# cloneofsimo/paint-with-words-sd

Measured on AMD Instinct MI355X. Metric: 512x512 images/sec (30 steps, CFG) SD1.5+PwW, higher is better.
Workload: dtype bf16

## Files before the change

__graft_entry__.py:

```python
import os
import sys

REPO = os.path.dirname(os.path.abspath(__file__))
PKG = os.path.join(REPO, "paint-with-words-sd_amd")
for p in (PKG, REPO, os.path.join(REPO, "tests")):
    if p not in sys.path:
        sys.path.insert(0, p)


def build():
    import build as pww_build
    lib = pww_build.build_lib(verbose=False)
    exe = pww_build.build_native_check()
    import pww_hip
    import paint_with_words
    handle = pww_hip.load_library()
    missing = [n for n in pww_hip.EXPORTS if not hasattr(handle, n)]
    assert not missing, "libpww_hip.so lacks %s" % missing
    from pww_hip import _lib
    built = [(lib, handle.pww_version())]
    for name in pww_build.SIDE_LIBS:
        path = pww_build.build_side(name)
        side = _lib.load_side(name)
        assert side is not None, "%s was not built" % path
        missing = [n for n in _lib.side_spec(name)["exports"] if not hasattr(side, n)]
        assert not missing, "%s lacks %s" % (os.path.basename(path), missing)
        built.append((path, getattr(side, "pww_%s_version" % name)()))
    print("built %s and %s" % (", ".join("%s (ABI %d)" % b for b in built), exe))


def smoke():
    import math
    import numpy as np
    import torch
    import pww_hip
    from oracle import pww_oracle as O
    import pww_cases as cases

    assert torch.cuda.is_available(), "smoke() needs a HIP device"
    dev = torch.device("cuda:0")
    print("device arch:", pww_hip.device_arch())

    case = cases.make_attention_case("sd15_n1024")
    dtype = torch.float16
    mod = case["attn_cross"].to(dev, dtype)
    hidden = case["hidden"].to(dev, dtype)
    wf = lambda w, sigma, qk: 0.4 * w * math.log(1 + sigma) * qk.max()
    ctx = {"CONTEXT_TENSOR": case["ctx"].to(dev, dtype), "CROSS_ATTENTION_WEIGHT_1024": case["w"].to(dev),
           "SIGMA": torch.tensor(7.84), "WEIGHT_FUNCTION": wf}
    y = pww_hip.inj_forward(mod, hidden, ctx).float().cpu()
# ... 35 lines not shown
```

paint-with-words-sd_amd/build.py:

```python
import os
import subprocess
import sys

HERE = os.path.dirname(os.path.abspath(__file__))
REPO = os.path.dirname(HERE)
CSRC = os.path.join(HERE, "csrc")
LIB = os.path.join(HERE, "pww_hip", "libpww_hip.so")
LIB_EXPERIMENTS = os.path.join(HERE, "pww_hip", "libpww_hip_experiments.so")
UNITS = [("pww_api.hip", [], ""), ("pww_attn.hip", [], ""), ("pww_cross.hip", [], ""), ("pww_cross_lean.hip", [], ""), ("pww_reduce.hip", [], ""),
         ("pww_mask.hip", [], ""), ("pww_qproj.hip", [], ""), ("pww_norm.hip", [], ""), ("pww_blocks.hip", [], ""), ("pww_conv.hip", [], ""), ("pww_probs.hip", [], ""),
         ("pww_attn_inst.hip", ["-DPWW_INST_F16"], ".f16"), ("pww_attn_inst.hip", ["-DPWW_INST_BF16"], ".bf16"),
         ("pww_cross_inst.hip", ["-DPWW_INST_F16", "-DPWW_INST_NW=2"], ".f16.nw2"), ("pww_cross_inst.hip", ["-DPWW_INST_F16", "-DPWW_INST_NW=4"], ".f16.nw4"),
         ("pww_cross_inst.hip", ["-DPWW_INST_BF16", "-DPWW_INST_NW=2"], ".bf16.nw2"), ("pww_cross_inst.hip", ["-DPWW_INST_BF16", "-DPWW_INST_NW=4"], ".bf16.nw4")]
EXPERIMENT_UNITS = [("pww_cross_out.hip", [], "")]
_ATTN_HEADERS = ["pww_tile.h", "pww_attn_core.h", "pww_cross_tile.h"]
SIDE_FLAGS = ["-fvisibility=hidden"]
SIDE_LIBS = {
    "long": ("pww_long.hip", _ATTN_HEADERS, "the long-prompt launches"),
    "scope": ("pww_scope.hip", _ATTN_HEADERS, "cross-attention with per-head / per-row score statistics"),
    "linear": ("pww_linear.hip", [], "linear layers with a bias / residual / GEGLU epilogue"),
    "regions": ("pww_regions.hip", [], "region masks and the per-pixel blend of the noise predictions"),
    "lora": ("pww_lora.hip", [], "the per-row low-rank update of unmerged LoRA adapters"),
}
SOURCES = sorted({u[0] for u in UNITS + EXPERIMENT_UNITS})
HEADERS = ["pww_common.h", "pww_tile.h", "pww_attn_core.h", "pww_attn_kernel.h", "pww_cross_tile.h", "pww_cross_kernel.h", os.path.join(REPO, "include", "pww_hip.h")]
SIDE_PATHS = {n: os.path.join(HERE, "pww_hip", "libpww_hip_%s.so" % n) for n in SIDE_LIBS}
SIDE_UNITS = {n: [(v[0], SIDE_FLAGS, "")] for n, v in SIDE_LIBS.items()}
LIB_LONG, LIB_SCOPE, LIB_LINEAR, LIB_REGIONS, LIB_LORA = (SIDE_PATHS[n] for n in ("long", "scope", "linear", "regions", "lora"))
LONG_UNITS, SCOPE_UNITS, LINEAR_UNITS, REGIONS_UNITS, LORA_UNITS = (SIDE_UNITS[n] for n in ("long", "scope", "linear", "regions", "lora"))
HIPCC = os.environ.get("HIPCC", "/opt/rocm/bin/hipcc")
FLAGS = ["--offload-arch=gfx950", "-O3", "-std=c++17", "-fPIC", "-Wall",
         "-Wno-unused-function", "-mllvm", "-amdgpu-kernarg-preload-count=16"]


PER_FILE_FLAGS = {"pww_mask.hip": ["-ffp-contract=off"], "pww_regions.hip": ["-ffp-contract=off"]}


def _newer(target, deps):
    if not os.path.exists(target):
        return True
    t = os.path.getmtime(target)
    return any(os.path.getmtime(d) > t for d in deps)


def _deps():
    return ([os.path.join(CSRC, s) for s in SOURCES] + [h if os.path.isabs(h) else os.path.join(CSRC, h) for h in HEADERS] + [__file__])


def _build(lib, units, defines, objdir, verbose, jobs=None):
    os.makedirs(objdir, exist_ok=True)
    order = sorted(units, key=lambda u: {"pww_cross_inst.hip": 0, "pww_attn_inst.hip": 1, "pww_cross_lean.hip": 2}.get(u[0], 3))
    jobs = jobs or max(2, min(len(order), os.cpu_count() or 4, int(os.environ.get("MAX_JOBS", 16))))
# ... 12 lines not shown
        if p.returncode != 0:
            for _, q in running:
                q.kill()
            raise RuntimeError("hipcc failed: %s\n%s" % (" ".join(cmd), out))
        if verbose and out.strip():
            print(out)
    subprocess.run([HIPCC, "--offload-arch=gfx950", "-shared", "-fPIC", "-s"] + sorted(objs) + ["-o", lib], check=True)
    return lib


def build_lib(force=False, verbose=False):
    if not force and not _newer(LIB, _deps()):
        return LIB
    return _build(LIB, UNITS, [], os.path.join(HERE, "build"), verbose)


def build_experiments(force=False, verbose=False):
    if not force and not _newer(LIB_EXPERIMENTS, _deps()):
        return LIB_EXPERIMENTS
    return _build(LIB_EXPERIMENTS, UNITS + EXPERIMENT_UNITS, ["-DPWW_EXPERIMENTS=1"], os.path.join(HERE, "build", "experiments"), verbose)


def build_side(name, force=False, verbose=False):
    unit, headers, _ = SIDE_LIBS[name]
    lib = SIDE_PATHS[name]
    deps = [os.path.join(CSRC, f) for f in [unit, "pww_common.h", "pww_side_host.h"] + headers] + [os.path.join(REPO, "include", h) for h in ("pww_hip.h", "pww_hip_%s.h" % name)] + [__file__]
    if not force and not _newer(lib, deps):
        return lib
    return _build(lib, SIDE_UNITS[name], [], os.path.join(HERE, "build", name), verbose)


def build_long(force=False, verbose=False): return build_side("long", force, verbose)
def build_scope(force=False, verbose=False): return build_side("scope", force, verbose)
def build_linear(force=False, verbose=False): return build_side("linear", force, verbose)
def build_regions(force=False, verbose=False): return build_side("regions", force, verbose)
def build_lora(force=False, verbose=False): return build_side("lora", force, verbose)


def _build_check(exe, lib, libname, defines, force):
    src = os.path.join(REPO, "tests", "native", "attn_check.cpp")
    if not force and not _newer(exe, [src, lib, os.path.join(REPO, "include", "pww_hip.h")]):
        return exe
    cmd = [HIPCC, "--offload-arch=gfx950", "-O2", "-std=c++17"] + defines + [src, "-o", exe, "-L" + os.path.dirname(lib), "-l" + libname,
                                                                              "-Wl,-rpath,$ORIGIN/../../paint-with-words-sd_amd/pww_hip"]
    subprocess.run(cmd, check=True)
    return exe


def build_native_check(force=False):
    return _build_check(os.path.join(REPO, "tests", "native", "attn_check"), build_lib(), "pww_hip", [], force)


def build_native_check_experiments(force=False):
    return _build_check(os.path.join(REPO, "tests", "native", "attn_check_experiments"), build_experiments(), "pww_hip_experiments", ["-DPWW_EXPERIMENTS=1"], force)


if __name__ == "__main__":
    force = "--force" in sys.argv
    print(build_lib(force=force, verbose=True))
    print(build_native_check(force=force))
    for name in SIDE_LIBS:
        print(build_side(name, force=force, verbose=True))
    if "--experiments" in sys.argv:
        print(build_experiments(force=force, verbose=True))
        print(build_native_check_experiments(force=force))
```

paint-with-words-sd_amd/pww_hip/_lib.py:

```python
import ctypes
import os

_HERE = os.path.dirname(os.path.abspath(__file__))
LIB_PATH = os.environ.get("PWW_HIP_LIB", os.path.join(_HERE, "libpww_hip.so"))
EXPERIMENTS_LIB_PATH = os.environ.get("PWW_HIP_EXPERIMENTS_LIB", os.path.join(_HERE, "libpww_hip_experiments.so"))

LONG_LIB_PATH = os.environ.get("PWW_HIP_LONG_LIB", os.path.join(_HERE, "libpww_hip_long.so"))
SCOPE_LIB_PATH = os.environ.get("PWW_HIP_SCOPE_LIB", os.path.join(_HERE, "libpww_hip_scope.so"))
LINEAR_LIB_PATH = os.environ.get("PWW_HIP_LINEAR_LIB", os.path.join(_HERE, "libpww_hip_linear.so"))
REGIONS_LIB_PATH = os.environ.get("PWW_HIP_REGIONS_LIB", os.path.join(_HERE, "libpww_hip_regions.so"))
LORA_LIB_PATH = os.environ.get("PWW_HIP_LORA_LIB", os.path.join(_HERE, "libpww_hip_lora.so"))

PWW_OK, PWW_EINVAL, PWW_ENOTSUP, PWW_EHIP = 0, -22, -95, -5
MIN_VERSION = 127
DTYPE_F16, DTYPE_BF16 = 0, 1
LAYOUT_NCHW, LAYOUT_NHWC = 0, 1
ACT_NONE, ACT_SILU = 0, 1
LINEAR_NONE, LINEAR_BIAS, LINEAR_BIAS_RESIDUAL, LINEAR_BIAS_GEGLU = 0, 1, 2, 3
MAX_HEAD_DIM = 160

EXPORTS = ("pww_version", "pww_has_experiments", "pww_last_error", "pww_device_arch", "pww_self_attn_fwd", "pww_cross_attn_fwd",
           "pww_cross_attn_fwd_stat", "pww_cross_attn_fwd_stat_ex",
           "pww_qk_reduce", "pww_mask_build", "pww_mask_build_rgb", "pww_mask_build_f32", "pww_resize_tokens", "pww_gauss_blur", "pww_inpaint_prep", "pww_cfg_combine", "pww_store_f32",
           "pww_workspace_bytes", "pww_profile_arm", "pww_profile_elapsed_us", "pww_profile_reset", "pww_debug_timeline", "pww_debug_path_counts",
           "pww_debug_last_attn_route",
           "pww_qproj_stat", "pww_qproj_parts", "pww_cross_attn_fwd_parts", "pww_mask_build_f32_levels", "pww_qk_parts", "pww_qk_parts_count",
           "pww_group_norm_fwd", "pww_group_norm_workspace_bytes", "pww_add_layer_norm", "pww_add_layer_norm_bias", "pww_geglu", "pww_bias_residual",
           "pww_conv3x3_workspace_bytes", "pww_conv3x3_fwd", "pww_cross_attn_probs")
EXPERIMENT_EXPORTS = ("pww_cross_attn_fwd_fused", "pww_cross_attn_fwd_fused_ex", "pww_cross_fused_workspace_bytes", "pww_cross_fused_state_bytes",
                      "pww_cross_attn_fwd_parts_out", "pww_cross_attn_out_supported")


LONG_EXPORTS = ("pww_long_version", "pww_long_last_error", "pww_long_qk_parts", "pww_long_qk_parts_count", "pww_long_cross_attn_fwd_parts",
                "pww_long_cross_attn_probs", "pww_long_profile_arm", "pww_long_profile_elapsed_us")
LONG_MIN_VERSION = 100
LONG_MIN_KEYS, LONG_MAX_KEYS = 129, 256


SCOPE_EXPORTS = ("pww_scope_version", "pww_scope_last_error", "pww_scope_head_parts_count", "pww_scope_head_parts", "pww_scope_cross_attn_fwd")
SCOPE_MIN_VERSION = 100
SCOPE_HEAD, SCOPE_ROW = 1, 2


LINEAR_EXPORTS = ("pww_linear_version", "pww_linear_last_error", "pww_linear_workspace_bytes", "pww_linear_fwd")
LINEAR_MIN_VERSION = 100


REGIONS_EXPORTS = ("pww_regions_version", "pww_regions_last_error", "pww_regions_masks", "pww_regions_combine")
REGIONS_MIN_VERSION = 100
REGIONS_MAX, REGIONS_MAX_PLANE, REGIONS_MAX_FEATHER = 8, 9216, 8.0


LORA_EXPORTS = ("pww_lora_version", "pww_lora_last_error", "pww_lora_fwd")
LORA_MIN_VERSION = 100
LORA_MAX_ADAPTERS, LORA_MAX_RANK, LORA_MAX_SEGMENTS = 8, 128, 3


class AttnDesc(ctypes.Structure):
    _fields_ = [("dtype", ctypes.c_int32), ("B", ctypes.c_int32), ("H", ctypes.c_int32), ("N", ctypes.c_int32),
                ("M", ctypes.c_int32), ("D", ctypes.c_int32),
                ("q_stride", ctypes.c_int64 * 3), ("k_stride", ctypes.c_int64 * 3),
                ("v_stride", ctypes.c_int64 * 3), ("o_stride", ctypes.c_int64 * 3),
                ("scale", ctypes.c_float), ("bias_stride", ctypes.c_int64 * 4)]


class CrossOpts(ctypes.Structure):
    _fields_ = [("size", ctypes.c_uint32), ("bias_cols", ctypes.c_int32), ("coeff_scalar_dev", ctypes.c_void_p),
                ("bias_compact", ctypes.c_void_p), ("col_idx", ctypes.c_void_p), ("R", ctypes.c_int32), ("gated_images", ctypes.c_int32),
                ("compact_stride", ctypes.c_int64 * 2), ("col_idx_stride", ctypes.c_int64)]


class QprojDesc(ctypes.Structure):
    _fields_ = [("dtype", ctypes.c_int32), ("B", ctypes.c_int32), ("N", ctypes.c_int32), ("Cin", ctypes.c_int32), ("H", ctypes.c_int32),
                ("D", ctypes.c_int32), ("M", ctypes.c_int32), ("x_stride", ctypes.c_int64 * 2), ("q_stride", ctypes.c_int64 * 2),
                ("k_stride", ctypes.c_int64 * 2)]


class GnDesc(ctypes.Structure):
    _fields_ = [("dtype", ctypes.c_int32), ("layout", ctypes.c_int32), ("B", ctypes.c_int32), ("C", ctypes.c_int32), ("HW", ctypes.c_int32),
                ("G", ctypes.c_int32), ("eps", ctypes.c_float), ("act", ctypes.c_int32), ("add_stride", ctypes.c_int32), ("_pad", ctypes.c_int32)]
# ... 5 lines not shown


class ConvDesc(ctypes.Structure):
    _fields_ = [("size", ctypes.c_uint32), ("dtype", ctypes.c_int32), ("B", ctypes.c_int32), ("Hin", ctypes.c_int32), ("Win", ctypes.c_int32),
                ("Cin", ctypes.c_int32), ("Cout", ctypes.c_int32), ("stride", ctypes.c_int32), ("upsample", ctypes.c_int32), ("tile_n", ctypes.c_int32),
                ("splitk", ctypes.c_int32), ("_pad", ctypes.c_int32)]


class LinearDesc(ctypes.Structure):
    _fields_ = [("size", ctypes.c_uint32), ("dtype", ctypes.c_int32), ("M", ctypes.c_int32), ("N", ctypes.c_int32), ("K", ctypes.c_int32),
                ("epilogue", ctypes.c_int32), ("x_stride", ctypes.c_int64), ("y_stride", ctypes.c_int64), ("r_stride", ctypes.c_int64),
                ("tile_n", ctypes.c_int32), ("splitk", ctypes.c_int32)]


class ProbsDesc(ctypes.Structure):
    _fields_ = [("size", ctypes.c_uint32), ("images", ctypes.c_int32), ("accumulate", ctypes.c_int32), ("weight", ctypes.c_float),
                ("out_stride", ctypes.c_int64 * 2)]


class LoraDesc(ctypes.Structure):
    _fields_ = [("size", ctypes.c_uint32), ("dtype", ctypes.c_int32), ("R", ctypes.c_int32), ("T", ctypes.c_int32), ("K", ctypes.c_int32),
                ("N", ctypes.c_int32), ("n_seg", ctypes.c_int32), ("rank", ctypes.c_int32), ("n_adapters", ctypes.c_int32), ("_pad", ctypes.c_int32),
                ("x_row_stride", ctypes.c_int64), ("x_tok_stride", ctypes.c_int64), ("y_row_stride", ctypes.c_int64), ("y_tok_stride", ctypes.c_int64)]


class Region(ctypes.Structure):
    _fields_ = [("r", ctypes.c_uint8), ("g", ctypes.c_uint8), ("b", ctypes.c_uint8), ("_pad", ctypes.c_uint8),
                ("strength", ctypes.c_float)]


class PwwHipError(RuntimeError):
    pass


_lib = None
_exp = None


def _bind(lib, experiments):
    vp, i32, i64, f32 = ctypes.c_void_p, ctypes.c_int32, ctypes.c_int64, ctypes.c_float
    lib.pww_version.restype = ctypes.c_int
    if lib.pww_version() // 100 != 1 or lib.pww_version() < MIN_VERSION:
        raise PwwHipError("libpww_hip ABI version %d.%02d is not 1.x >= 1.%02d (rebuild: python paint-with-words-sd_amd/build.py)"
                          % (lib.pww_version() // 100, lib.pww_version() % 100, MIN_VERSION % 100))
    lib.pww_last_error.restype = ctypes.c_char_p
    lib.pww_device_arch.argtypes = [ctypes.c_char_p, ctypes.c_size_t]
# ... 119 lines not shown
SIDE = {
    "long": dict(path="LONG_LIB_PATH", exports=LONG_EXPORTS, min_version=LONG_MIN_VERSION, missing_ok=False, needs="prompts longer than 77 tokens need it", sigs={
        "pww_long_qk_parts": ([_vp, _vp, _vp, _P(AttnDesc), _i32, _i32, _vp, _sz, _vp], _int),
        "pww_long_qk_parts_count": ([_P(AttnDesc)], _i32),
        "pww_long_cross_attn_fwd_parts": ([_vp, _vp, _vp, _vp, _vp, _i32, _f32, _vp, _P(AttnDesc), _vp, _i32, _vp, _P(CrossOpts), _vp], _int),
        "pww_long_cross_attn_probs": ([_vp, _vp, _vp, _vp, _i32, _f64, _f32, _vp, _P(AttnDesc), _P(CrossOpts), _vp, _P(ProbsDesc), _vp], _int),
        "pww_long_profile_arm": ([], _int),
        "pww_long_profile_elapsed_us": ([_P(_f32)], _int)}),
    "scope": dict(path="SCOPE_LIB_PATH", exports=SCOPE_EXPORTS, min_version=SCOPE_MIN_VERSION, missing_ok=True, needs="per-head / per-row score statistics need it", sigs={
        "pww_scope_head_parts_count": ([_P(AttnDesc)], _i32),
        "pww_scope_head_parts": ([_vp, _vp, _vp, _P(AttnDesc), _i32, _vp, _sz, _vp], _int),
        "pww_scope_cross_attn_fwd": ([_vp, _vp, _vp, _vp, _vp, _i32, _i32, _f32, _vp, _P(AttnDesc), _vp, _i32, _vp, _P(CrossOpts), _vp], _int)}),
    "linear": dict(path="LINEAR_LIB_PATH", exports=LINEAR_EXPORTS, min_version=LINEAR_MIN_VERSION, missing_ok=False, needs="linear layers on the native kernel need it", sigs={
        "pww_linear_workspace_bytes": ([_P(LinearDesc)], _sz),
        "pww_linear_fwd": ([_vp, _vp, _vp, _vp, _vp, _P(LinearDesc), _vp, _sz, _vp], _int)}),
    "regions": dict(path="REGIONS_LIB_PATH", exports=REGIONS_EXPORTS, min_version=REGIONS_MIN_VERSION, missing_ok=False, needs="region prompts need it", sigs={
        "pww_regions_masks": ([_vp, _i32, _i32, _vp, _i32, _f32, _vp, _vp], _int),
        "pww_regions_combine": ([_vp, _vp, _vp, _vp, _f32, _vp, _i32, _i32, _i32, _i64, _i32, _vp], _int)}),
}
SIDE_MORE = {
    "lora": dict(path="LORA_LIB_PATH", exports=LORA_EXPORTS, min_version=LORA_MIN_VERSION, missing_ok=False, needs="LoRA adapters on the native kernel need it", sigs={
        "pww_lora_fwd": ([_vp, _vp, _vp, _vp, _vp, _vp, _P(LoraDesc), _vp], _int)}),
}
_side = {}


def side_spec(name):
    return SIDE[name] if name in SIDE else SIDE_MORE[name]


def load_side(name):
    lib = _side.get(name)
    if lib is not None:
        return lib
    spec = side_spec(name)
    path, so, pre = globals()[spec["path"]], "libpww_hip_%s.so" % name, "pww_%s_" % name
    if not os.path.isfile(path):
        if spec["missing_ok"]:
            return None
        raise PwwHipError("%s not found at %s: %s %s" % (so, path, spec["needs"], _HINT))
    try:
        lib = ctypes.CDLL(path)
        getattr(lib, pre + "version").restype = _int
        version = getattr(lib, pre + "version")()
    except (OSError, AttributeError) as e:
        raise PwwHipError("%s at %s cannot be loaded: %s %s" % (so, path, e, _HINT))
    if version // 100 != 1 or version < spec["min_version"]:
        raise PwwHipError("%s ABI version %d is not 1.x >= %d %s" % (so[:-3], version, spec["min_version"], _HINT))
    missing = [n for n in spec["exports"] if not hasattr(lib, n)]
    if missing:
        raise PwwHipError("%s at %s lacks %s %s" % (so, path, missing, _HINT))
# ... 10 lines not shown
    return lib if lib is not None else load_side("long")


def load_scope():
    lib = _side.get("scope")
    return lib if lib is not None else load_side("scope")


def load_linear():
    lib = _side.get("linear")
    return lib if lib is not None else load_side("linear")


def load_regions():
    lib = _side.get("regions")
    return lib if lib is not None else load_side("regions")


def load_lora():
    lib = _side.get("lora")
    return lib if lib is not None else load_side("lora")


class experiments:

    def __enter__(self):
        global _lib
        load()
        self._prev = _lib
        _lib = load_experiments()
        return _lib

    def __exit__(self, *exc):
        global _lib
        _lib = self._prev
        return False


def check(rc, what, lib=None):
    if rc != PWW_OK:
        msg = (lib or load()).pww_last_error().decode("utf-8", "replace")
        raise PwwHipError("%s failed (rc=%d): %s" % (what, rc, msg))


def device_arch():
    buf = ctypes.create_string_buffer(64)
# ... 3 lines not shown
```

paint-with-words-sd_amd/pww_hip/blocks.py:

```python
import os
import types
import warnings

import torch
import torch.nn as nn
import torch.nn.functional as F

from . import ops

FUSED_NORM = os.environ.get("PWW_FUSED_NORM", "1") != "0"
BATCHED_TEMB = os.environ.get("PWW_BATCHED_TEMB", "1") != "0"
FOLD_CONV_BIAS = os.environ.get("PWW_FOLD_CONV_BIAS", "1") != "0"
CONV1X1_AS_LINEAR = os.environ.get("PWW_CONV1X1_AS_LINEAR", "1") != "0"
LINEAR = os.environ.get("PWW_LINEAR", "1")
CONV3X3 = os.environ.get("PWW_CONV3X3", "1") != "0"


_STATS = {k: [0, 0] for k in ("group_norm", "resnet_block", "transformer_block", "geglu", "conv1x1", "conv3x3", "linear")}
_UNRATED = ("conv1x1", "conv3x3", "linear")
_warned = set()


def stats():
    out = {k: {"fused": v[0], "declined": v[1]} for k, v in _STATS.items()}
    rated = [v for k, v in _STATS.items() if k not in _UNRATED]
    tot = sum(v[0] + v[1] for v in rated)
    out["hit_rate"] = (sum(v[0] for v in rated) / tot) if tot else None
    return out


def reset_stats():
    for v in _STATS.values():
        v[0] = v[1] = 0


def _count(op, fused, x=None, reason=None):
    _STATS[op][0 if fused else 1] += 1
    if not fused and FUSED_NORM and torch.is_tensor(x) and x.is_cuda and x.dtype in (torch.float16, torch.bfloat16):
        key = (op, reason)
        if key not in _warned:
            _warned.add(key)
            warnings.warn("pww_hip.blocks: %s call on a HIP %s tensor handed to the stock op (%s); pww_hip.blocks.stats() counts them"
# ... 106 lines not shown
    h = fused_group_norm(self.norm1, input_tensor, act="silu")
    if fold and _conv3x3_route(self.conv1, h):
        h = ops.conv3x3(h, self.conv1.weight)
    else:
        h = _conv_no_bias(self.conv1, h) if fold else self.conv1(h)
    add = None
    if temb is not None and getattr(self, "time_emb_proj", None) is not None:
        slot = self.__dict__.get("_pww_temb_slot")
        if slot is not None and temb.dtype == h.dtype and temb.dim() == 2 and not torch.is_grad_enabled():
            add = slot[0].project(temb)[:, slot[1]:slot[1] + slot[2]]
        else:
            add = self.time_emb_proj(F.silu(temb))
        if add.dtype != h.dtype:
            add = add.to(h.dtype)
    if fold and _takes(h, self.norm2):
        h = ops.group_norm(h, self.norm2.num_groups, self.norm2.weight, self.norm2.bias, self.norm2.eps, add=add, act="silu", pre_bias=self.conv1.bias)
    else:
        if fold:
            h = h + self.conv1.bias[None, :, None, None]
        h = fused_group_norm(self.norm2, h, add=add, act="silu")
    dropout = getattr(self, "dropout", None)
    if dropout is not None:
        h = dropout(h)
    if getattr(self, "conv_shortcut", None) is not None:
        input_tensor = self.conv_shortcut(input_tensor)
    scale = getattr(self, "output_scale_factor", 1.0)
    if fold and input_tensor.dtype == h.dtype and input_tensor.shape == (h.shape[0], self.conv2.out_channels) + h.shape[2:] and _conv3x3_route(self.conv2, h):
        out = ops.conv3x3(h, self.conv2.weight, self.conv2.bias, residual=input_tensor)
    elif fold and input_tensor.dtype == h.dtype and input_tensor.shape[1] % 8 == 0:
        out = ops.bias_residual(input_tensor, _conv_no_bias(self.conv2, h), self.conv2.bias)
    else:
        out = input_tensor + self.conv2(h)
    return out if scale == 1.0 else out / scale


def _is_conv3x3(m):
    return (isinstance(m, nn.Conv2d) and type(m).forward is nn.Conv2d.forward and m.kernel_size == (3, 3) and m.stride in ((1, 1), (2, 2))
            and m.padding == (1, 1) and m.dilation == (1, 1) and m.groups == 1 and m.padding_mode == "zeros")


STOCK_FROM_ROWS = 16384


def _conv3x3_route(conv, x, upsample=False):
    ok = (CONV3X3 and FUSED_NORM and torch.is_tensor(x) and x.dim() == 4 and _is_conv3x3(conv) and not torch.is_autocast_enabled() and not (torch.is_grad_enabled() and (x.requires_grad or conv.weight.requires_grad))
          and (conv.bias is None or conv.bias.dtype == x.dtype) and ops.conv3x3_takes(x, conv.weight, conv.stride[0], upsample)
          and (upsample or x.shape[0] * ((x.shape[2] - 1) // conv.stride[0] + 1) * ((x.shape[3] - 1) // conv.stride[0] + 1) < STOCK_FROM_ROWS))
    _STATS["conv3x3"][0 if ok else 1] += 1
    return ok


def _conv3x3_forward(self, x, *args, **kwargs):
    if not args and not kwargs and _conv3x3_route(self, x):
        return ops.conv3x3(x, self.weight, self.bias, stride=self.stride[0])
    return self._pww_orig_forward(x, *args, **kwargs)


def _upsample_conv(m):
    if getattr(m, "use_conv_transpose", False) or not getattr(m, "use_conv", True):
        return None
    conv = getattr(m, "Conv2d_0", None) if getattr(m, "name", "conv") != "conv" else getattr(m, "conv", None)
    return conv if _is_conv3x3(conv) and conv.stride == (1, 1) and "forward" not in conv.__dict__ and not conv._forward_hooks and not conv._forward_pre_hooks else None


def _upsample_forward(self, *args, **kwargs):
    plain = 1 <= len(args) <= 2 and set(kwargs) <= {"output_size"} and all(a is None for a in list(args[1:]) + list(kwargs.values()))
    x = args[0] if plain and not (len(args) == 2 and kwargs) else None
    conv = _upsample_conv(self)
    if x is not None and conv is not None and x.dim() == 4 and (getattr(self, "channels", None) in (None, x.shape[1])) and _conv3x3_route(conv, x, upsample=True):
        return ops.conv3x3(x, conv.weight, conv.bias, upsample=True)
    return self._pww_orig_forward(*args, **kwargs)
# ... 148 lines not shown
```

paint-with-words-sd_amd/pww_hip/ops.py:

```python
import ctypes

import torch

from . import _lib
from ._lib import AttnDesc, CrossOpts, ProbsDesc, QprojDesc, Region, PwwHipError

_DT = {torch.float16: _lib.DTYPE_F16, torch.bfloat16: _lib.DTYPE_BF16}


def _stream():
    return ctypes.c_void_p(torch.cuda.current_stream().cuda_stream)


def _ptr(t):
    return ctypes.c_void_p(t.data_ptr()) if t is not None else ctypes.c_void_p(0)


def _require_gpu(*tensors):
    for t in tensors:
        if t is not None and not t.is_cuda:
            raise PwwHipError("pww_hip ops need tensors on a HIP device (got %s); there is no CPU path" % t.device)


def _rows_ok(t):
# ... 919 lines not shown
    B, C, H, W = x.shape
    Cout = weight.shape[0]
    Hv, Wv = H << int(bool(upsample)), W << int(bool(upsample))
    Ho, Wo = (Hv - 1) // stride + 1, (Wv - 1) // stride + 1
    w = _khwc_weight(weight)
    if bias is not None and (bias.dtype != x.dtype or tuple(bias.shape) != (Cout,)):
        raise PwwHipError("conv3x3: bias must be a %s [%d]" % (x.dtype, Cout))
    if bias is not None:
        bias = bias.contiguous()
    if residual is not None:
        if tuple(residual.shape) != (B, Cout, Ho, Wo) or residual.dtype != x.dtype:
            raise PwwHipError("conv3x3: residual must be a %s %s" % (x.dtype, (B, Cout, Ho, Wo)))
        residual = residual.contiguous(memory_format=torch.channels_last)
    d = _lib.ConvDesc(ctypes.sizeof(_lib.ConvDesc), _DT[x.dtype], B, H, W, C, Cout, int(stride), int(bool(upsample)), int(tile_n), int(splitk), 0)
    lib = _lib.load()
    y = torch.empty((B, Cout, Ho, Wo), dtype=x.dtype, device=x.device, memory_format=torch.channels_last)
    nbytes = int(lib.pww_conv3x3_workspace_bytes(ctypes.byref(d)))
    ws = torch.empty(nbytes // 4, dtype=torch.float32, device=x.device) if nbytes else None
    with torch.cuda.device(x.device):
        _lib.check(lib.pww_conv3x3_fwd(_ptr(x), _ptr(w), _ptr(bias), _ptr(residual), _ptr(y), ctypes.byref(d), _ptr(ws), nbytes, _stream()), "pww_conv3x3_fwd")
    return y


def _linear_weight(weight):
    if not torch.is_tensor(weight) or weight.dim() not in (2, 4) or (weight.dim() == 4 and tuple(weight.shape[2:]) != (1, 1)):
        return None
    w = weight.detach().reshape(weight.shape[0], weight.shape[1]) if weight.dim() == 4 else weight.detach()
    return w if w.is_contiguous() and w.data_ptr() == weight.data_ptr() and w.data_ptr() % 16 == 0 else None


def linear_takes(x, weight, geglu=False, bias=None, residual=None, out=None):
    if not (torch.is_tensor(x) and x.is_cuda and x.dtype in _DT and x.dim() >= 2 and torch.is_tensor(weight) and weight.dtype == x.dtype):
        return False
    w = _linear_weight(weight)
    if w is None or x.shape[-1] != w.shape[1] or x.numel() == 0 or _rows(x, "linear") is None:
        return False
    N, K = w.shape
    rows, _, xs = _rows(x, "linear")
    if not (K % 64 == 0 and N % (128 if geglu else 64) == 0 and rows * xs < 2 ** 31 and rows * N < 2 ** 31 and N * K < 2 ** 31):
        return False
    if bias is not None and not (torch.is_tensor(bias) and bias.is_cuda and bias.dtype == x.dtype and tuple(bias.shape) == (N,) and bias.is_contiguous()
                                 and bias.data_ptr() % 8 == 0):
        return False
    shape = tuple(x.shape[:-1]) + (N // 2 if geglu else N,)
    for t in (residual, out):
        if t is not None and not (torch.is_tensor(t) and t.is_cuda and t.dtype == x.dtype and tuple(t.shape) == shape and _rows(t, "linear") is not None):
# ... 100 lines not shown
```

Before: 5.104.

## Fuse ResnetBlock 1x1 conv shortcut into conv2 as extra K-slabs

Adds a new side library with an implicit-GEMM 3x3 conv kernel that treats the 1x1 conv shortcut as additional K-slabs, so conv2 and the shortcut projection are computed in one accumulation with both biases added in the epilogue. This removes the separate shortcut GEMM launch and the write and reread of its output as a residual. It adds split-K with an fp32 workspace and a fold kernel, per-shape tuned tile and split tables, and a routing check in the ResnetBlock forward that falls back to the old path when conditions are not met.

```diff
diff --git a/__graft_entry__.py b/__graft_entry__.py
--- a/__graft_entry__.py
+++ b/__graft_entry__.py
@@ -19,13 +19,18 @@
     assert not missing, "libpww_hip.so lacks %s" % missing
     from pww_hip import _lib
     built = [(lib, handle.pww_version())]
-    for name in pww_build.SIDE_LIBS:
+    def build_side(name):
         path = pww_build.build_side(name)
         side = _lib.load_side(name)
         assert side is not None, "%s was not built" % path
         missing = [n for n in _lib.side_spec(name)["exports"] if not hasattr(side, n)]
         assert not missing, "%s lacks %s" % (os.path.basename(path), missing)
         built.append((path, getattr(side, "pww_%s_version" % name)()))
+
+    for name in pww_build.SIDE_LIBS:
+        build_side(name)
+    for name in pww_build.SIDE_LIBS_CONV:
+        build_side(name)
     print("built %s and %s" % (", ".join("%s (ABI %d)" % b for b in built), exe))
 
 
diff --git a/include/pww_hip_convtail.h b/include/pww_hip_convtail.h
--- /dev/null
+++ b/include/pww_hip_convtail.h
@@ -0,0 +1,30 @@
+#ifndef PWW_HIP_CONVTAIL_H
+#define PWW_HIP_CONVTAIL_H
+
+#include "pww_hip.h"
+
+#ifdef __cplusplus
+extern "C" {
+#endif
+
+#define PWW_CONVTAIL_VERSION 100
+
+int pww_convtail_version(void);
+const char *pww_convtail_last_error(void);
+
+typedef struct pww_convtail_desc {
+    uint32_t size;
+    int32_t dtype;
+    int32_t B, H, W;
+    int32_t Cin, C2, Cout;
+    int32_t tile_n, splitk;
+} pww_convtail_desc_t;
+size_t pww_convtail_workspace_bytes(const pww_convtail_desc_t *desc);
+int pww_convtail_fwd(const void *x, const void *w, const void *x2, const void *w2, const void *bias, const void *bias2, void *y,
+                     const pww_convtail_desc_t *desc, void *workspace, size_t workspace_bytes, void *stream);
+
+#ifdef __cplusplus
+}
+#endif
+
+#endif
diff --git a/paint-with-words-sd_amd/build.py b/paint-with-words-sd_amd/build.py
--- a/paint-with-words-sd_amd/build.py
+++ b/paint-with-words-sd_amd/build.py
@@ -22,12 +22,17 @@
     "regions": ("pww_regions.hip", [], "region masks and the per-pixel blend of the noise predictions"),
     "lora": ("pww_lora.hip", [], "the per-row low-rank update of unmerged LoRA adapters"),
 }
+SIDE_LIBS_CONV = {
+    "convtail": ("pww_conv_tail.hip", [], "conv2 of a ResnetBlock2D with the 1 x 1 shortcut as further K-slabs"),
+}
+ALL_SIDE_LIBS = {**SIDE_LIBS, **SIDE_LIBS_CONV}
 SOURCES = sorted({u[0] for u in UNITS + EXPERIMENT_UNITS})
 HEADERS = ["pww_common.h", "pww_tile.h", "pww_attn_core.h", "pww_attn_kernel.h", "pww_cross_tile.h", "pww_cross_kernel.h", os.path.join(REPO, "include", "pww_hip.h")]
-SIDE_PATHS = {n: os.path.join(HERE, "pww_hip", "libpww_hip_%s.so" % n) for n in SIDE_LIBS}
-SIDE_UNITS = {n: [(v[0], SIDE_FLAGS, "")] for n, v in SIDE_LIBS.items()}
+SIDE_PATHS = {n: os.path.join(HERE, "pww_hip", "libpww_hip_%s.so" % n) for n in ALL_SIDE_LIBS}
+SIDE_UNITS = {n: [(v[0], SIDE_FLAGS, "")] for n, v in ALL_SIDE_LIBS.items()}
 LIB_LONG, LIB_SCOPE, LIB_LINEAR, LIB_REGIONS, LIB_LORA = (SIDE_PATHS[n] for n in ("long", "scope", "linear", "regions", "lora"))
 LONG_UNITS, SCOPE_UNITS, LINEAR_UNITS, REGIONS_UNITS, LORA_UNITS = (SIDE_UNITS[n] for n in ("long", "scope", "linear", "regions", "lora"))
+LIB_CONVTAIL, CONVTAIL_UNITS = SIDE_PATHS["convtail"], SIDE_UNITS["convtail"]
 HIPCC = os.environ.get("HIPCC", "/opt/rocm/bin/hipcc")
 FLAGS = ["--offload-arch=gfx950", "-O3", "-std=c++17", "-fPIC", "-Wall",
          "-Wno-unused-function", "-mllvm", "-amdgpu-kernarg-preload-count=16"]
@@ -86,7 +91,7 @@
 
 
 def build_side(name, force=False, verbose=False):
-    unit, headers, _ = SIDE_LIBS[name]
+    unit, headers, _ = ALL_SIDE_LIBS[name]
     lib = SIDE_PATHS[name]
     deps = [os.path.join(CSRC, f) for f in [unit, "pww_common.h", "pww_side_host.h"] + headers] + [os.path.join(REPO, "include", h) for h in ("pww_hip.h", "pww_hip_%s.h" % name)] + [__file__]
     if not force and not _newer(lib, deps):
@@ -99,6 +104,7 @@
 def build_linear(force=False, verbose=False): return build_side("linear", force, verbose)
 def build_regions(force=False, verbose=False): return build_side("regions", force, verbose)
 def build_lora(force=False, verbose=False): return build_side("lora", force, verbose)
+def build_convtail(force=False, verbose=False): return build_side("convtail", force, verbose)
 
 
 def _build_check(exe, lib, libname, defines, force):
@@ -123,7 +129,7 @@
     force = "--force" in sys.argv
     print(build_lib(force=force, verbose=True))
     print(build_native_check(force=force))
-    for name in SIDE_LIBS:
+    for name in ALL_SIDE_LIBS:
         print(build_side(name, force=force, verbose=True))
     if "--experiments" in sys.argv:
         print(build_experiments(force=force, verbose=True))
diff --git a/paint-with-words-sd_amd/csrc/pww_conv_tail.hip b/paint-with-words-sd_amd/csrc/pww_conv_tail.hip
--- /dev/null
+++ b/paint-with-words-sd_amd/csrc/pww_conv_tail.hip
@@ -0,0 +1,296 @@
+#define PWW_SIDE_LIB "libpww_hip_convtail"
+#include "pww_side_host.h"
+#include "../../include/pww_hip_convtail.h"
+
+#define PWW_CONVTAIL_API extern "C" __attribute__((visibility("default")))
+
+namespace pww {
+
+namespace {
+
+constexpr int CT_BM = 128, CT_THREADS = 256;
+constexpr int CT_PF = 2;
+
+__device__ __forceinline__ f32x4 mfma16(f16x8 a, f16x8 b, f32x4 c) { return __builtin_amdgcn_mfma_f32_16x16x32_f16(a, b, c, 0, 0, 0); }
+__device__ __forceinline__ f32x4 mfma16(bf16x8 a, bf16x8 b, f32x4 c) { return __builtin_amdgcn_mfma_f32_16x16x32_bf16(a, b, c, 0, 0, 0); }
+
+struct TailCold {
+    const void *x2, *w2, *bias, *bias2;
+    int nsplit, nmain, ntail;
+};
+
+__device__ __forceinline__ int xcd_remap(int orig, int nwg) {
+    const int xcd = orig & 7, q = nwg >> 3, r = nwg & 7;
+    return (xcd < r ? xcd * (q + 1) : r * (q + 1) + (xcd - r) * q) + (orig >> 3);
+}
+
+template <typename T>
+__device__ __forceinline__ void epilogue4(const f32x4 &a, const TailCold &cold, T *y, long off, int n) {
+    typedef typename Vec<T>::v4 V4;
+    const V4 b = *reinterpret_cast<const V4 *>(reinterpret_cast<const T *>(cold.bias) + n);
+    const V4 b2 = *reinterpret_cast<const V4 *>(reinterpret_cast<const T *>(cold.bias2) + n);
+    V4 o;
+#pragma unroll
+    for (int j = 0; j < 4; ++j) o[j] = (T)(a[j] + (float)b[j] + (float)b2[j]);
+    *reinterpret_cast<V4 *>(y + off) = o;
+}
+
+template <typename T, int BN>
+__global__ void __launch_bounds__(CT_THREADS, 2) convtail_kernel(const T *__restrict__ x, const T *__restrict__ w, void *__restrict__ out, int M, int N,
+                                                                 int Cin, int C2, int H, int W, const TailCold cold) {
+    typedef typename Vec<T>::v8 V8;
+    constexpr int BM = CT_BM, PF = CT_PF, XL = BM * 8 / CT_THREADS, WL = BN * 8 / CT_THREADS, RM = 4, RN = BN / 32;
+    constexpr int XBYTES = BM * 128, STAGE = (BM + BN) * 128;
+    __shared__ __attribute__((aligned(16))) char lds[2 * STAGE];
+
+    const int tid = threadIdx.x, lane = tid & 63, wave = tid >> 6, wm = wave >> 1, wn = wave & 1;
+    const int ntm = (M + BM - 1) / BM;
+    const int bid = xcd_remap(blockIdx.x, gridDim.x);
+    const bool split = cold.nsplit > 1;
+    const int tile = bid / cold.nsplit, ks = bid - tile * cold.nsplit;
+    const int tm = tile % ntm, tn = tile / ntm;
+    const int nmain = cold.nmain, nslab = nmain + cold.ntail;
+    const int s_begin = (int)((long)ks * nslab / cold.nsplit), s_end = (int)((long)(ks + 1) * nslab / cold.nsplit);
+    const int K9 = 9 * Cin, HW = H * W;
+    const T *__restrict__ x2 = reinterpret_cast<const T *>(cold.x2);
+    const T *__restrict__ w2 = reinterpret_cast<const T *>(cold.w2);
+
+    const int c = tid & 7;
+    int pix[XL], y0[XL], x0[XL];
+#pragma unroll
+    for (int i = 0; i < XL; ++i) {
+        int m = tm * BM + (tid >> 3) + 32 * i;
+        m = m < M ? m : M - 1;
+        const int b = m / HW, rem = m - b * HW, oy = rem / W, ox = rem - oy * W;
+        pix[i] = b * HW;
+        y0[i] = oy - 1;
+        x0[i] = ox - 1;
+    }
+    const unsigned wrow = (unsigned)(tn * BN + (tid >> 3));
+    const unsigned woff_main = wrow * (unsigned)K9 + c * 8, woff_tail = wrow * (unsigned)C2 + c * 8;
+    const int swz = ((c ^ ((tid >> 3) & 7)) << 4);
+
+    u32x4 xr[PF][XL], wr[PF][WL];
+    unsigned xok[PF];
+    const bool tail0 = s_begin >= nmain;
+    int tap = tail0 ? 9 : s_begin / (Cin >> 6);
+    int ci0 = tail0 ? (s_begin - nmain) << 6 : (s_begin - tap * (Cin >> 6)) << 6;
+    int kmain = s_begin * 64;
+    auto load = [&](int p) {
+        const bool tail = tap >= 9;
+        const int ky = tail ? 1 : tap / 3, kx = tail ? 1 : tap - (tap / 3) * 3;
+        const T *xb = tail ? x2 : x;
+        const T *wb = tail ? w2 : w;
+        const int pitch = tail ? C2 : Cin;
+        const unsigned wpitch = (unsigned)(tail ? C2 : K9);
+        const unsigned wo = (tail ? woff_tail : woff_main) + (unsigned)(tail ? ci0 : kmain);
+        xok[p] = 0;
+#pragma unroll
+        for (int i = 0; i < XL; ++i) {
+            const int iy = y0[i] + ky, ix = x0[i] + kx;
+            const bool ok = (unsigned)iy < (unsigned)H && (unsigned)ix < (unsigned)W;
+            xr[p][i] = *reinterpret_cast<const u32x4 *>(xb + (unsigned)((pix[i] + (ok ? iy : 0) * W + (ok ? ix : 0)) * pitch + ci0 + c * 8));
+            xok[p] |= (unsigned)ok << i;
+        }
+#pragma unroll
+        for (int j = 0; j < WL; ++j) wr[p][j] = *reinterpret_cast<const u32x4 *>(wb + (wo + (unsigned)(32 * j) * wpitch));
+        kmain += 64;
+        ci0 += 64;
+        const bool wrap = ci0 == Cin && !tail;
+        ci0 = wrap ? 0 : ci0;
+        tap += wrap ? 1 : 0;
+    };
+    auto store = [&](int p, int buf) {
+        char *base = lds + buf * STAGE;
+#pragma unroll
+        for (int i = 0; i < XL; ++i) {
+            const u32x4 z = {0u, 0u, 0u, 0u};
+            *reinterpret_cast<u32x4 *>(base + ((tid >> 3) + 32 * i) * 128 + swz) = (xok[p] >> i) & 1u ? xr[p][i] : z;
+        }
+#pragma unroll
+        for (int j = 0; j < WL; ++j) *reinterpret_cast<u32x4 *>(base + XBYTES + ((tid >> 3) + 32 * j) * 128 + swz) = wr[p][j];
+    };
+
+    f32x4 acc[RN][RM];
+#pragma unroll
+    for (int r = 0; r < RN; ++r)
+#pragma unroll
+        for (int i = 0; i < RM; ++i) acc[r][i] = f32x4{0.f, 0.f, 0.f, 0.f};
+
+    const int fr = lane & 15, fq = lane >> 4;
+    auto compute = [&](int buf) {
+        const char *bx = lds + buf * STAGE, *bw = bx + XBYTES;
+#pragma unroll
+        for (int kk = 0; kk < 2; ++kk) {
+            V8 xf[RM], wf[RN];
+#pragma unroll
+            for (int q = 0; q < RM; ++q) {
+                const int row = wm * 64 + q * 16 + fr;
+                xf[q] = *reinterpret_cast<const V8 *>(bx + row * 128 + (((kk * 4 + fq) ^ (row & 7)) << 4));
+            }
+#pragma unroll
+            for (int r = 0; r < RN; ++r) {
+                const int row = wn * (BN / 2) + r * 16 + fr;
+                wf[r] = *reinterpret_cast<const V8 *>(bw + row * 128 + (((kk * 4 + fq) ^ (row & 7)) << 4));
+            }
+#pragma unroll
+            for (int r = 0; r < RN; ++r)
+#pragma unroll
+                for (int q = 0; q < RM; ++q) acc[r][q] = mfma16(wf[r], xf[q], acc[r][q]);
+        }
+    };
+
+    const int n = s_end - s_begin;
+    load(0);
+#pragma unroll
+    for (int p = 1; p < PF; ++p)
+        if (p < n) load(p);
+    store(0, 0);
+    __syncthreads();
+    int i = 0;
+    for (; i + 2 * PF <= n; i += PF) {
+#pragma unroll
+        for (int p = 0; p < PF; ++p) {
+            load(p);
+            compute((i + p) & 1);
+            __builtin_amdgcn_sched_barrier(0);
+            store((p + 1) % PF, (i + p + 1) & 1);
+            __syncthreads();
+        }
+    }
+#pragma unroll
+    for (int t = 0; t < 2 * PF - 1; ++t) {
+        if (i + t < n) {
+            if (i + t + PF < n) load(t % PF);
+            compute((i + t) & 1);
+            if (i + t + 1 < n) store((t + 1) % PF, (i + t + 1) & 1);
+            __syncthreads();
+        }
+    }
+
+#pragma unroll
+    for (int i = 0; i < RM; ++i) {
+        const int m = tm * BM + wm * 64 + i * 16 + fr;
+        if (m >= M) continue;
+#pragma unroll
+        for (int r = 0; r < RN; ++r) {
+            const int n = tn * BN + wn * (BN / 2) + r * 16 + fq * 4;
+            if (split) *reinterpret_cast<f32x4 *>(reinterpret_cast<float *>(out) + ((long)ks * M + m) * N + n) = acc[r][i];
+            else epilogue4<T>(acc[r][i], cold, reinterpret_cast<T *>(out), (long)m * N + n, n);
+        }
+    }
+}
+
+template <typename T>
+__global__ void __launch_bounds__(256) convtail_fold_kernel(const float *__restrict__ ws, T *__restrict__ y, long n4, int N, long MN, const TailCold cold) {
+    const long q = (long)blockIdx.x * 256 + threadIdx.x;
+    if (q >= n4) return;
+    const long off = q * 4;
+    f32x4 a = *reinterpret_cast<const f32x4 *>(ws + off);
+    for (int s = 1; s < cold.nsplit; ++s) a += *reinterpret_cast<const f32x4 *>(ws + s * MN + off);
+    epilogue4<T>(a, cold, y, off, (int)(off % N));
+}
+
+struct TailTune { int M, N, nmain, ntail, bn, nsplit; };
+constexpr TailTune TAIL_TUNED[] = {
+    {128, 1280, 180, 40, 64, 12},
+    {512, 1280, 180, 40, 128, 12}, {512, 1280, 180, 30, 128, 12}, {512, 1280, 180, 10, 128, 12},
+    {2048, 640, 90, 30, 128, 6}, {2048, 640, 90, 20, 128, 6}, {2048, 640, 90, 15, 128, 6}, {2048, 640, 90, 5, 128, 6},
+    {8192, 320, 45, 15, 64, 4}, {8192, 320, 45, 10, 64, 4},
+};
+
+struct TailPlan {
+    int M, bn, nsplit, nmain, ntail, ntiles;
+};
+
+bool plan_tail(const pww_convtail_desc_t *d, TailPlan *p) {
+    if (!d || d->size < sizeof(pww_convtail_desc_t)) { set_error("convtail: descriptor missing or older than this library (size %u)", d ? d->size : 0u); return false; }
+    if ((d->dtype != PWW_DTYPE_F16 && d->dtype != PWW_DTYPE_BF16) || d->B < 1 || d->H < 1 || d->W < 1 || d->Cin < 64 || d->Cin % 64 != 0 || d->C2 < 64
+        || d->C2 % 64 != 0 || d->Cout < 64 || d->Cout % 64 != 0 || d->Cin > 65536 || d->C2 > 65536 || d->Cout > 65536) {
+        set_error("convtail: unsupported (dtype %d B %d %dx%d Cin %d C2 %d Cout %d): Cin, C2 and Cout multiples of 64", d->dtype, d->B, d->H, d->W, d->Cin,
+                  d->C2, d->Cout);
+        return false;
+    }
+    const long M = (long)d->B * d->H * d->W;
+    if (M * d->Cin >= (1L << 31) || M * d->C2 >= (1L << 31) || M * d->Cout >= (1L << 31) || 9L * d->Cin * d->Cout >= (1L << 31)
+        || (long)d->C2 * d->Cout >= (1L << 31)) {
+        set_error("convtail: tensor of 2^31 elements or more");
+        return false;
+    }
+    p->M = (int)M;
+    p->nmain = 9 * d->Cin / 64;
+    p->ntail = d->C2 / 64;
+    const int nslab = p->nmain + p->ntail;
+    const TailTune *tuned = nullptr;
+    for (const TailTune &t : TAIL_TUNED)
+        if (t.M == p->M && t.N == d->Cout && t.nmain == p->nmain && t.ntail == p->ntail) tuned = &t;
+    p->bn = d->tile_n ? d->tile_n : tuned ? tuned->bn : (d->Cout % 128 == 0 ? 128 : 64);
+    if ((p->bn != 64 && p->bn != 128) || d->Cout % p->bn != 0) { set_error("convtail: tile_n %d does not divide Cout %d", d->tile_n, d->Cout); return false; }
+    p->ntiles = (p->M + CT_BM - 1) / CT_BM * (d->Cout / p->bn);
+    int ns = d->splitk;
+    if (ns <= 0 && tuned && p->bn == tuned->bn) ns = tuned->nsplit;
+    if (ns <= 0) {
+        ns = (480 + p->ntiles / 2) / p->ntiles;
+        if (ns > nslab / 8) ns = nslab / 8;
+        if (ns < 1) ns = 1;
+    }
+    if (ns > nslab || ns > 64) { set_error("convtail: split %d exceeds the %d K-slabs (or 64)", ns, nslab); return false; }
+    p->nsplit = ns;
+    return true;
+}
+
+template <typename T>
+int tail_launch(const TailPlan &p, const pww_convtail_desc_t *d, const void *x, const void *w, const void *x2, const void *w2, const void *bias,
+                const void *bias2, void *y, void *ws, hipStream_t stream) {
+    TailCold cold{x2, w2, bias, bias2, p.nsplit, p.nmain, p.ntail};
+    const T *xt = static_cast<const T *>(x), *wt = static_cast<const T *>(w);
+    const int N = d->Cout;
+    const dim3 grid(p.ntiles * p.nsplit), block(CT_THREADS);
+    void *out = p.nsplit == 1 ? y : ws;
+    if (p.bn == 128) launch_timed(convtail_kernel<T, 128>, grid, block, 0, stream, xt, wt, out, p.M, N, d->Cin, d->C2, d->H, d->W, cold);
+    else launch_timed(convtail_kernel<T, 64>, grid, block, 0, stream, xt, wt, out, p.M, N, d->Cin, d->C2, d->H, d->W, cold);
+    if (p.nsplit == 1) return check_hip(hipGetLastError(), "convtail launch");
+    const long MN = (long)p.M * N, n4 = MN / 4;
+    launch_timed(convtail_fold_kernel<T>, dim3((unsigned)((n4 + 255) / 256)), dim3(256), 0, stream, static_cast<const float *>(ws), static_cast<T *>(y), n4,
+                 N, MN, cold);
+    return check_hip(hipGetLastError(), "convtail fold launch");
+}
+
+}
+
+size_t convtail_workspace_bytes(const pww_convtail_desc_t *d) {
+    TailPlan p;
+    if (!plan_tail(d, &p)) return 0;
+    return p.nsplit > 1 ? (size_t)p.nsplit * p.M * d->Cout * sizeof(float) : 0;
+}
+
+int convtail_fwd(const void *x, const void *w, const void *x2, const void *w2, const void *bias, const void *bias2, void *y, const pww_convtail_desc_t *d,
+                 void *workspace, size_t workspace_bytes, hipStream_t stream) {
+    if (!d || d->size < sizeof(pww_convtail_desc_t)) { set_error("convtail: descriptor missing or older than this library (size %u)", d ? d->size : 0u); return PWW_EINVAL; }
+    TailPlan p;
+    if (!plan_tail(d, &p)) return PWW_ENOTSUP;
+    if (!x || !w || !x2 || !w2 || !bias || !bias2 || !y) { set_error("convtail: x, w, x2, w2, bias, bias2 and y are required"); return PWW_EINVAL; }
+    if (!aligned16(x) || !aligned16(w) || !aligned16(x2) || !aligned16(w2) || !aligned16(y) || (reinterpret_cast<uintptr_t>(bias) & 7)
+        || (reinterpret_cast<uintptr_t>(bias2) & 7)) {
+        set_error("convtail: x, w, x2, w2, y must be 16-byte aligned, the biases 8-byte aligned");
+        return PWW_EINVAL;
+    }
+    const size_t need = p.nsplit > 1 ? (size_t)p.nsplit * p.M * d->Cout * sizeof(float) : 0;
+    if (need && (!workspace || !aligned16(workspace) || workspace_bytes < need)) {
+        set_error("convtail: split %d needs a 16-byte aligned workspace of %zu bytes (got %zu)", p.nsplit, need, workspace_bytes);
+        return PWW_EINVAL;
+    }
+    if (!arch_ok()) return PWW_ENOTSUP;
+    if (d->dtype == PWW_DTYPE_F16) return tail_launch<f16>(p, d, x, w, x2, w2, bias, bias2, y, workspace, stream);
+    return tail_launch<bf16>(p, d, x, w, x2, w2, bias, bias2, y, workspace, stream);
+}
+
+}
+
+PWW_CONVTAIL_API int pww_convtail_version(void) { return PWW_CONVTAIL_VERSION; }
+PWW_CONVTAIL_API const char *pww_convtail_last_error(void) { return pww::last_error(); }
+PWW_CONVTAIL_API size_t pww_convtail_workspace_bytes(const pww_convtail_desc_t *desc) { return pww::convtail_workspace_bytes(desc); }
+PWW_CONVTAIL_API int pww_convtail_fwd(const void *x, const void *w, const void *x2, const void *w2, const void *bias, const void *bias2, void *y,
+                                      const pww_convtail_desc_t *desc, void *workspace, size_t workspace_bytes, void *stream) {
+    return pww::convtail_fwd(x, w, x2, w2, bias, bias2, y, desc, workspace, workspace_bytes, static_cast<hipStream_t>(stream));
+}
diff --git a/paint-with-words-sd_amd/pww_hip/_lib.py b/paint-with-words-sd_amd/pww_hip/_lib.py
--- a/paint-with-words-sd_amd/pww_hip/_lib.py
+++ b/paint-with-words-sd_amd/pww_hip/_lib.py
@@ -10,6 +10,7 @@
 LINEAR_LIB_PATH = os.environ.get("PWW_HIP_LINEAR_LIB", os.path.join(_HERE, "libpww_hip_linear.so"))
 REGIONS_LIB_PATH = os.environ.get("PWW_HIP_REGIONS_LIB", os.path.join(_HERE, "libpww_hip_regions.so"))
 LORA_LIB_PATH = os.environ.get("PWW_HIP_LORA_LIB", os.path.join(_HERE, "libpww_hip_lora.so"))
+CONVTAIL_LIB_PATH = os.environ.get("PWW_HIP_CONVTAIL_LIB", os.path.join(_HERE, "libpww_hip_convtail.so"))
 
 PWW_OK, PWW_EINVAL, PWW_ENOTSUP, PWW_EHIP = 0, -22, -95, -5
 MIN_VERSION = 127
@@ -56,6 +57,10 @@
 LORA_MAX_ADAPTERS, LORA_MAX_RANK, LORA_MAX_SEGMENTS = 8, 128, 3
 
 
+CONVTAIL_EXPORTS = ("pww_convtail_version", "pww_convtail_last_error", "pww_convtail_workspace_bytes", "pww_convtail_fwd")
+CONVTAIL_MIN_VERSION = 100
+
+
 class AttnDesc(ctypes.Structure):
     _fields_ = [("dtype", ctypes.c_int32), ("B", ctypes.c_int32), ("H", ctypes.c_int32), ("N", ctypes.c_int32),
                 ("M", ctypes.c_int32), ("D", ctypes.c_int32),
@@ -107,6 +112,11 @@
     _fields_ = [("size", ctypes.c_uint32), ("dtype", ctypes.c_int32), ("R", ctypes.c_int32), ("T", ctypes.c_int32), ("K", ctypes.c_int32),
                 ("N", ctypes.c_int32), ("n_seg", ctypes.c_int32), ("rank", ctypes.c_int32), ("n_adapters", ctypes.c_int32), ("_pad", ctypes.c_int32),
                 ("x_row_stride", ctypes.c_int64), ("x_tok_stride", ctypes.c_int64), ("y_row_stride", ctypes.c_int64), ("y_tok_stride", ctypes.c_int64)]
+
+
+class ConvTailDesc(ctypes.Structure):
+    _fields_ = [("size", ctypes.c_uint32), ("dtype", ctypes.c_int32), ("B", ctypes.c_int32), ("H", ctypes.c_int32), ("W", ctypes.c_int32),
+                ("Cin", ctypes.c_int32), ("C2", ctypes.c_int32), ("Cout", ctypes.c_int32), ("tile_n", ctypes.c_int32), ("splitk", ctypes.c_int32)]
 
 
 class Region(ctypes.Structure):
@@ -272,11 +282,16 @@
     "lora": dict(path="LORA_LIB_PATH", exports=LORA_EXPORTS, min_version=LORA_MIN_VERSION, missing_ok=False, needs="LoRA adapters on the native kernel need it", sigs={
         "pww_lora_fwd": ([_vp, _vp, _vp, _vp, _vp, _vp, _P(LoraDesc), _vp], _int)}),
 }
+SIDE_CONV = {
+    "convtail": dict(path="CONVTAIL_LIB_PATH", exports=CONVTAIL_EXPORTS, min_version=CONVTAIL_MIN_VERSION, missing_ok=True, needs="conv2 with the shortcut as K-slabs needs it", sigs={
+        "pww_convtail_workspace_bytes": ([_P(ConvTailDesc)], _sz),
+        "pww_convtail_fwd": ([_vp, _vp, _vp, _vp, _vp, _vp, _vp, _P(ConvTailDesc), _vp, _sz, _vp], _int)}),
+}
 _side = {}
 
 
 def side_spec(name):
-    return SIDE[name] if name in SIDE else SIDE_MORE[name]
+    return SIDE[name] if name in SIDE else SIDE_MORE[name] if name in SIDE_MORE else SIDE_CONV[name]
 
 
 def load_side(name):
@@ -333,6 +348,11 @@
     return lib if lib is not None else load_side("lora")
 
 
+def load_convtail():
+    lib = _side.get("convtail")
+    return lib if lib is not None else load_side("convtail")
+
+
 class experiments:
 
     def __enter__(self):
diff --git a/paint-with-words-sd_amd/pww_hip/blocks.py b/paint-with-words-sd_amd/pww_hip/blocks.py
--- a/paint-with-words-sd_amd/pww_hip/blocks.py
+++ b/paint-with-words-sd_amd/pww_hip/blocks.py
@@ -14,10 +14,11 @@
 CONV1X1_AS_LINEAR = os.environ.get("PWW_CONV1X1_AS_LINEAR", "1") != "0"
 LINEAR = os.environ.get("PWW_LINEAR", "1")
 CONV3X3 = os.environ.get("PWW_CONV3X3", "1") != "0"
-
-
-_STATS = {k: [0, 0] for k in ("group_norm", "resnet_block", "transformer_block", "geglu", "conv1x1", "conv3x3", "linear")}
-_UNRATED = ("conv1x1", "conv3x3", "linear")
+CONV_SHORTCUT = os.environ.get("PWW_CONV_SHORTCUT", "1") != "0"
+
+
+_STATS = {k: [0, 0] for k in ("group_norm", "resnet_block", "transformer_block", "geglu", "conv1x1", "conv3x3", "linear", "conv_shortcut")}
+_UNRATED = ("conv1x1", "conv3x3", "linear", "conv_shortcut")
 _warned = set()
 
 
@@ -170,9 +171,12 @@
     dropout = getattr(self, "dropout", None)
     if dropout is not None:
         h = dropout(h)
-    if getattr(self, "conv_shortcut", None) is not None:
-        input_tensor = self.conv_shortcut(input_tensor)
     scale = getattr(self, "output_scale_factor", 1.0)
+    shortcut = getattr(self, "conv_shortcut", None)
+    if shortcut is not None:
+        if _conv_shortcut_route(self, shortcut, h, input_tensor, fold, scale):
+            return ops.conv3x3_shortcut(h, self.conv2.weight, self.conv2.bias, input_tensor, shortcut.weight, shortcut.bias)
+        input_tensor = shortcut(input_tensor)
     if fold and input_tensor.dtype == h.dtype and input_tensor.shape == (h.shape[0], self.conv2.out_channels) + h.shape[2:] and _conv3x3_route(self.conv2, h):
         out = ops.conv3x3(h, self.conv2.weight, self.conv2.bias, residual=input_tensor)
     elif fold and input_tensor.dtype == h.dtype and input_tensor.shape[1] % 8 == 0:
@@ -195,6 +199,23 @@
           and (conv.bias is None or conv.bias.dtype == x.dtype) and ops.conv3x3_takes(x, conv.weight, conv.stride[0], upsample)
           and (upsample or x.shape[0] * ((x.shape[2] - 1) // conv.stride[0] + 1) * ((x.shape[3] - 1) // conv.stride[0] + 1) < STOCK_FROM_ROWS))
     _STATS["conv3x3"][0 if ok else 1] += 1
+    return ok
+
+
+def _conv_shortcut_route(block, shortcut, h, x, fold, scale):
+    own = shortcut.__dict__.get("forward")
+    ok = (CONV_SHORTCUT and fold and scale == 1.0 and _is_conv1x1(shortcut) and shortcut.bias is not None
+          and (own is None or getattr(own, "__func__", None) is _conv1x1_forward) and not shortcut._forward_hooks and not shortcut._forward_pre_hooks
+          and torch.is_tensor(x) and x.dim() == 4 and x.dtype == h.dtype == shortcut.weight.dtype == shortcut.bias.dtype
+          and x.is_contiguous(memory_format=torch.channels_last)
+          and not (torch.is_grad_enabled() and (x.requires_grad or shortcut.weight.requires_grad))
+          and _is_conv3x3(block.conv2) and block.conv2.stride == (1, 1) and ops.conv3x3_shortcut_takes(h, block.conv2.weight, x, shortcut.weight)
+          and ops._lib.load_convtail() is not None)
+    if ok:
+        ok = _conv3x3_route(block.conv2, h)
+        if not ok:
+            _STATS["conv3x3"][1] -= 1
+    _STATS["conv_shortcut"][0 if ok else 1] += 1
     return ok
 
 
diff --git a/paint-with-words-sd_amd/pww_hip/ops.py b/paint-with-words-sd_amd/pww_hip/ops.py
--- a/paint-with-words-sd_amd/pww_hip/ops.py
+++ b/paint-with-words-sd_amd/pww_hip/ops.py
@@ -965,6 +965,43 @@
     return y
 
 
+def conv3x3_shortcut_takes(h, conv2_weight, x, shortcut_weight):
+    if not (conv3x3_takes(h, conv2_weight) and torch.is_tensor(x) and x.is_cuda and x.device == h.device and x.dim() == 4 and x.dtype == h.dtype
+            and torch.is_tensor(shortcut_weight) and shortcut_weight.dtype == h.dtype and shortcut_weight.device == h.device):
+        return False
+    w2 = _linear_weight(shortcut_weight)
+    B, C2, H, W = x.shape
+    return (w2 is not None and tuple(w2.shape) == (conv2_weight.shape[0], C2) and C2 % 64 == 0 and (B, H, W) == (h.shape[0], h.shape[2], h.shape[3])
+            and x.is_contiguous(memory_format=torch.channels_last) and x.data_ptr() % 16 == 0 and B * H * W * C2 < 2 ** 31 // 4)
+
+
+def conv3x3_shortcut(h, conv2_weight, conv2_bias, x, shortcut_weight, shortcut_bias, tile_n=0, splitk=0):
+    _require_gpu(h, conv2_weight, conv2_bias, x, shortcut_weight, shortcut_bias)
+    if not conv3x3_shortcut_takes(h, conv2_weight, x, shortcut_weight):
+        raise PwwHipError("conv3x3_shortcut: needs channels_last float16/bfloat16 h and x of one dtype, batch and size, channel counts multiples of 64, "
+                          "a 3 x 3 weight and a dense 1 x 1 weight of that dtype")
+    B, C, H, W = h.shape
+    Cout, C2 = conv2_weight.shape[0], x.shape[1]
+    w = _khwc_weight(conv2_weight)
+    w2 = _linear_weight(shortcut_weight)
+    biases = []
+    for name, b in (("conv2_bias", conv2_bias), ("shortcut_bias", shortcut_bias)):
+        if not torch.is_tensor(b) or b.dtype != h.dtype or tuple(b.shape) != (Cout,):
+            raise PwwHipError("conv3x3_shortcut: %s must be a %s [%d]" % (name, h.dtype, Cout))
+        biases.append(b.contiguous() if b.data_ptr() % 8 == 0 else b.clone(memory_format=torch.contiguous_format))
+    lib = _lib.load_convtail()
+    if lib is None:
+        raise PwwHipError("conv3x3_shortcut: libpww_hip_convtail.so is not built %s" % _lib._HINT)
+    d = _lib.ConvTailDesc(ctypes.sizeof(_lib.ConvTailDesc), _DT[h.dtype], B, H, W, C, C2, Cout, int(tile_n), int(splitk))
+    y = torch.empty((B, Cout, H, W), dtype=h.dtype, device=h.device, memory_format=torch.channels_last)
+    nbytes = int(lib.pww_convtail_workspace_bytes(ctypes.byref(d)))
+    ws = torch.empty(nbytes // 4, dtype=torch.float32, device=h.device) if nbytes else None
+    with torch.cuda.device(h.device):
+        _lib.check(lib.pww_convtail_fwd(_ptr(h), _ptr(w), _ptr(x), _ptr(w2), _ptr(biases[0]), _ptr(biases[1]), _ptr(y), ctypes.byref(d), _ptr(ws), nbytes,
+                                        _stream()), "pww_convtail_fwd", lib)
+    return y
+
+
 def _linear_weight(weight):
     if not torch.is_tensor(weight) or weight.dim() not in (2, 4) or (weight.dim() == 4 and tuple(weight.shape[2:]) != (1, 1)):
         return None
```

Result: faster. 5.216, median of 6 (+2.2%).
